# TencentARC/TVTS

Measured on AMD Instinct MI355X. Metric: video-text pairs/sec/node, TVTSv2 pretrain step, higher is better.
Workload: dtype bf16; 1 GPU; TVTSv2 ViT-B/16 8-frame 224^2, mask 0.5, 32-token captions x4, full pretrain step (fwd+losses+bwd+HF-AdamW); pairs_per_gpu=192, global_batch=192, parallelism=dp1, hip_graph=False

## Files before the change

include/tvts_hip.h:

```cpp
#ifndef TVTS_HIP_H
#define TVTS_HIP_H
#include <hip/hip_runtime_api.h>
#ifdef __cplusplus
extern "C" {
#endif

enum { TVTS_ACT_NONE = 0, TVTS_ACT_QUICK_GELU = 1, TVTS_ACT_GELU_ERF = 2,
       TVTS_GATE_ADD_BF16 = 3  };
enum { TVTS_ATTN_FULL = 0, TVTS_ATTN_SPACE = 1, TVTS_ATTN_TIME = 2, TVTS_ATTN_CLS = 3 };
enum {
    TVTS_GEMM_TILE_128 = 1,
    TVTS_GEMM_TILE_256 = 2,
    TVTS_GEMM_FP8_K32 = 4,
    TVTS_TN_NO_EARLY_DMA = 4,
    TVTS_TN_AFAST_0 = 8,
    TVTS_TN_AFAST_1 = 16,
    TVTS_GEMM_STREAMK = 32,
    TVTS_GEMM_NO_STREAMK = 64,
    TVTS_GEMM_RING = 128,
    TVTS_GEMM_NO_RING = 16384,
    TVTS_GEMM_F32_PATCH = 4194304,
    TVTS_GEMM_CLOCK_SAMPLE = 2097152,
    TVTS_GEMM_SIDE_DERIV = 1048576
};
#define TVTS_GEMM_RING_ROWS(r) ((r) == 128 ? (1 << 16) : (r) == 192 ? (2 << 16) : (r) == 256 ? (3 << 16) : 0)
#define TVTS_GEMM_CUS(n) ((((n) / 8) & 63) << 8)
#define TVTS_TN_SPLITS(s) ((s) << 8)
enum {
    TVTS_ATTN_NO_TR = 1,
    TVTS_ATTN_NO_SHARED = 2,
    TVTS_ATTN_NO_FUSED = 4
};

int tvts_gemm_nt_bf16(const void* A, int lda, const void* B, int ldb, int M, int N, int K, const float* bias,
                      const float* residual, int ldr, int act, void* preact, int ldp, const void* gate_h, int ldh,
                      int gate_act, void* out, int ldc, int out_f32, void* workspace, long workspace_bytes, int opts,
                      hipStream_t stream);
long tvts_gemm_nt_workspace_bytes(void);
int tvts_gemm_nt_select(int M, int N, int opts);
int tvts_gemm_tn_bf16(const void* P, int ldp, const void* Q, int ldq, int M, int Na, int Nb, float* out, int ldo,
                      int accumulate, float* colsum, float* workspace, long workspace_elems, int* counters, int n_counters,
                      int opts, hipStream_t stream);
int tvts_gemm_tn_bf16_grouped(const void* problems, int n, void* table_dev, void* table_host, long table_bytes, int upload,
                              float* workspace, long workspace_elems, int opts, hipStream_t stream);
long tvts_gemm_tn_grouped_table_bytes(int n);
int tvts_gemm_tn_select(int M, int Na, int Nb, int opts);
int tvts_gemm_nt_fp8(const void* A, int lda, const void* B, int ldb, int M, int N, int K, const float* scale_a,
                     int scale_a_rows, const float* scale_b, const float* bias, const float* residual, int ldr, int act, void* preact, int ldp,
                     void* out, int ldc, int out_f32, void* q8out, int ldq8, const float* q8_scale, float* q8_amax, int opts,
                     hipStream_t stream);
int tvts_gemm_nt_fp8_gate(const void* A, int lda, const void* B, int ldb, int M, int N, int K, const float* scale_a,
                          int scale_a_rows, const float* scale_b, const float* bias, const void* gate_h, int ldh, int gate_act,
                          void* out, int ldc, void* q8out, int ldq8, const float* q8_scale, float* q8_amax, int opts,
                          hipStream_t stream);
int tvts_gemm_tn_fp8(const void* P8, int ldp, const void* Q8, int ldq, int M, int Na, int Nb, const float* scale_p,
                     const float* scale_q, float* out, int ldo, int accumulate, float* colsum, float* workspace,
                     long workspace_elems, int opts, hipStream_t stream);
int tvts_amax(const void* x, int is_f32, long ld, int rows, int cols, float* amax, hipStream_t stream);
int tvts_quant_fp8(const void* x, int is_f32, long ld, int rows, int cols, const float* amax, void* out, long ldo,
                   float* scale_out, hipStream_t stream);
int tvts_quant_fp8_multi(const void* table, int n, hipStream_t stream);
int tvts_quant_fp8_rows(const void* x, long ld, int rows, int cols, void* out, long ldo, float* row_scale,
                        const float* tscale, float* amax_acc, hipStream_t stream);
int tvts_fp8_update_scales(float* amax, float* scale, int n, hipStream_t stream);
int tvts_gemm_small_f32(const float* A, long sai, long sak, const float* B, long sbk, long sbj, int M, int N, int K,
                        float alpha, const float* bias, float* C, long ldc, int accumulate, hipStream_t stream);
int tvts_rows_linear_bf16(const void* A, long lda, const void* W, int ldw, int R, int N, int K, const float* bias, const float* residual,
                          int ldr, float* out, int ldo, hipStream_t stream);
int tvts_colsum_bf16(const void* X, int ld, int M, int N, float* out, float* workspace, long workspace_elems, hipStream_t stream);

int tvts_layernorm_fwd(const void* x, int ldx, int x_bf16, const int* rows, const float* gamma, const float* beta, float eps, int M,
                       int W, void* y, int ldy, int y_f32, float* mean, float* rstd, hipStream_t stream);
int tvts_layernorm_fwd_fp8(const void* x, int ldx, int x_bf16, const int* rows, const float* gamma, const float* beta, float eps,
                           int M, int W, void* y, int ldy, void* q8, int ldq, float* row_scale, const float* tscale, float* amax_acc,
                           float* mean, float* rstd, hipStream_t stream);
int tvts_layernorm_bwd(const void* dy, int lddy, int dy_f32, const void* x, int ldx, int x_bf16, const int* rows, const float* mean,
                       const float* rstd, const float* gamma, const void* res1, int res1_bf16, int ldr, const void* res2_bf16, int ldr2,
                       int M, int W, float* dx, int lddx, void* dx_bf16, int lddxb, float* dgamma, float* dbeta,
                       float* workspace, long workspace_elems, hipStream_t stream);
int tvts_layernorm_bwd_fp8(const void* dy, int lddy, const void* x, int ldx, int x_bf16, const float* mean, const float* rstd,
                           const float* gamma, const void* res1, int res1_bf16, int ldr, const void* res2_bf16, int ldr2, int M, int W, float* dx,
                           int lddx, void* dx_bf16, int lddxb, void* q8, int ldq, float* row_scale, const float* tscale, float* amax_acc,
                           float* dgamma, float* dbeta, float* workspace, long workspace_elems, hipStream_t stream);
int tvts_layernorm_fwd_cls(const void* x, int ldx, const float* cls_x, int cls_period, void* x_refresh, const float* gamma,
                           const float* beta, float eps, int M, int W, void* y, int ldy, void* q8, int ldq, float* row_scale,
                           const float* tscale, float* amax_acc, float* mean, float* rstd, hipStream_t stream);
int tvts_layernorm_bwd_cls(const void* dy, int lddy, const void* x, int ldx, const float* cls_x, const float* cls_res1, float* cls_dx,
                           int cls_period, const float* mean, const float* rstd, const float* gamma, const void* res1_bf16, int ldr,
                           const void* res2_bf16, int ldr2, int M, int W, void* dx_bf16, int lddxb, void* q8, int ldq, float* row_scale,
                           const float* tscale, float* amax_acc, float* dgamma, float* dbeta, float* workspace, long workspace_elems,
                           hipStream_t stream);

int tvts_attn_fwd(int mode, const void* qkv, int ld, int B, int heads, int S, int T, int n, int causal, void* out, int ldo,
                  float* lse2, int opts, hipStream_t stream);
int tvts_attn_delta(const void* dO, int lddo, const void* O, int ldo, int rows, int heads, float* delta,
                    hipStream_t stream);
int tvts_attn_bwd_dq(int mode, const void* qkv, int ld, int B, int heads, int S, int T, int n, int causal, const void* dO,
                     int lddo, const float* lse2, const float* delta, void* dqkv, int lddq, int opts, hipStream_t stream);
int tvts_attn_bwd_dkv(int mode, const void* qkv, int ld, int B, int heads, int S, int T, int n, int causal, const void* dO,
                      int lddo, const float* lse2, const float* delta, void* dqkv, int lddq, float* cls_acc, int opts,
                      hipStream_t stream);
int tvts_attn_cls_finalize(const float* cls_acc, int B, int heads, int S, void* dqkv, int lddq, hipStream_t stream);
int tvts_attn_bwd(int mode, const void* qkv, int ld, int B, int heads, int S, int T, int n, int causal, const void* dO,
              int lddo, const void* O, int ldo, const float* lse2, float* delta, void* dqkv, int lddq, float* cls_acc,
              long cls_acc_elems, int opts, hipStream_t stream);
int tvts_attn_fwd_divided(int mode, const void* qkv, int ld, int B, int heads, int S, int T, int n, void* out, int ldo,
                      float* lse2, float* cls_ws, long cls_ws_elems, int opts, hipStream_t stream);
int tvts_attn_fwd_divided_q8(int mode, const void* qkv, int ld, int B, int heads, int S, int T, int n, void* out, int ldo,
                      float* lse2, float* cls_ws, long cls_ws_elems, void* q8out, int ldq8, const float* q8_scale, float* q8_amax,
                      int opts, hipStream_t stream);
int tvts_attn_bwd_q8(int mode, const void* qkv, int ld, int B, int heads, int S, int T, int n, int causal, const void* dO,
              int lddo, const void* O, int ldo, const float* lse2, float* delta, void* dqkv, int lddq, float* cls_acc,
              long cls_acc_elems, void* q8out, int ldq8, const float* q8_scale, float* q8_amax, int opts, hipStream_t stream);

// ... 121 lines not shown
```

tvts_amd/csrc/attention.hip:

```cpp
#include "common.h"
#include <stdlib.h>

enum { MODE_FULL = 0, MODE_SPACE = 1, MODE_TIME = 2, MODE_CLS = 3 };
#ifndef TVTS_DH
#define TVTS_DH 64
#endif
#define DH TVTS_DH
#if TVTS_DH == 64
#define NS_DH dh64
#define ABI(name) tvts_attn_##name
#define VSTRIDE 160
#else
#define NS_DH dh80
#define ABI(name) tvts_attn80_##name
#define VSTRIDE 192
#endif
namespace NS_DH {
constexpr int DT = DH / 16;
constexpr int KS = (DH + 31) / 32;
constexpr int NCH = DH / 8;

struct AttnGeom {
    int B, heads, S, T, n;
    int causal;
// ... 1706 lines not shown
                    for (int ks = 0; ks < KS; ++ks) sc = __builtin_amdgcn_mfma_f32_16x16x32_bf16(kc[t][ks], qc[qt][ks], sc, 0, 0, 0);
#pragma unroll
                    for (int e = 0; e < 4; ++e) {
                        const int key = t * 16 + gq * 4 + e;
                        const bool ok = key < m && !(key == 0 && qj == 0 && !first);
                        const float v = ok ? sc[e] * g.scale2 : -INFINITY;
                        st[t][e] = v;
                        mx = fmaxf(mx, v);
                    }
                }
            }
            mx = group_max(mx);
            float rs = 0.f;
#pragma unroll
            for (int t = 0; t < 2 * NU; ++t)
#pragma unroll
                for (int e = 0; e < 4; ++e) {
                    const float pp = __builtin_amdgcn_exp2f(st[t][e] - mx);
                    st[t][e] = pp;
                    rs += pp;
                }
            const float l = group_sum(rs);
            f32x4 o[DT];
#pragma unroll
            for (int dt = 0; dt < DT; ++dt) o[dt] = (f32x4){0, 0, 0, 0};
#pragma unroll
            for (int u = 0; u < NU; ++u) {
                bf16x8 pf;
#pragma unroll
                for (int j = 0; j < 8; ++j) pf[j] = (bf16)st[2 * u + (j >> 2)][j & 3];
#pragma unroll
                for (int dt = 0; dt < DT; ++dt)
                    o[dt] = __builtin_amdgcn_mfma_f32_16x16x32_bf16(frag_T_lim<TR>(Vs, u, dt, lane, RA, RS), pf, o[dt], 0, 0, 0);
            }
            {
                const float inv = 1.0f / l;
                f32x4 on[DT];
#pragma unroll
                for (int dt = 0; dt < DT; ++dt) on[dt] = o[dt] * inv;
                store_tile_rows(opatch, on, lane, [&](int rr) -> bf16* {
                    const int j = qt * 16 + rr;
                    return (j >= 1 && j < m) ? out + (size_t)k_row<MODE_TIME>(g, r, j) * ldo + hcol : nullptr; }, &q8o);
            }
            if (qj >= 1 && qj < m && gq == 0) lse2[(size_t)k_row<MODE_TIME>(g, r, qj) * g.heads + r.h] = mx + log2f(l);
            if (qt == 0) {
                const float Mn = fmaxf(Mr, mx);
                const float a = __builtin_amdgcn_exp2f(Mr - Mn), b = __builtin_amdgcn_exp2f(mx - Mn);
                Lr = Lr * a + l * b;
#pragma unroll
                for (int dt = 0; dt < DT; ++dt) Or[dt] = Or[dt] * a + o[dt] * b;
                Mr = Mn;
            }
        }
    }
    q8o.finish(g, lane);
    float* cst = (float*)(smem + wave * WB + TB);
    if (li == 0) {
        if (gq == 0) { cst[0] = Mr; cst[1] = Lr; }
#pragma unroll
        for (int dt = 0; dt < DT; ++dt)
#pragma unroll
            for (int e = 0; e < 4; ++e) cst[2 + dt * 16 + gq * 4 + e] = Or[dt][e];
    }
    __syncthreads();
    if (threadIdx.x < DH) {
        const int d = threadIdx.x;
        float M = -1e30f;
#pragma unroll
        for (int w = 0; w < 4; ++w) M = fmaxf(M, *(const float*)(smem + w * WB + TB));
        float L = 0.f, O = 0.f;
#pragma unroll
        for (int w = 0; w < 4; ++w) {
            const float* cw = (const float*)(smem + w * WB + TB);
            const float sc = __builtin_amdgcn_exp2f(cw[0] - M);
            L += cw[1] * sc;
            O += cw[2 + d] * sc;
        }
        float* cp = cls_part + ((size_t)(r.b * g.heads + r.h) * chunks + c) * (DH + 2);
        if (d == 0) { cp[0] = M; cp[1] = L; }
        cp[2 + d] = O;
    }
}

template <int MT, bool TR>
__global__ __launch_bounds__(256) void attn_fwd_seq_fused_kernel(AttnGeom g, const bf16* __restrict__ qkv,
                                                                 bf16* __restrict__ out, int ldo, float* __restrict__ lse2) {
    extern __shared__ __attribute__((aligned(16))) char smem[];
    constexpr int RA = MT * 16, TB = RA * VSTRIDE, NU = (MT + 1) / 2;
    constexpr int WB = TB + 1024;
    constexpr int PT = (RA * NCH + 63) / 64;
    const int lane = threadIdx.x & 63, wave = threadIdx.x >> 6;
    char* Vs = smem + wave * WB;
    char* opatch = Vs + TB;
    const int gq = lane >> 4, li = lane & 15;
    const int m = g.S, groups = g.B * g.heads, stride = gridDim.x * 4;
    const bool causal = g.causal != 0;

    bf16x8 qf[MT][KS], kf[MT][KS], vst[PT];
    auto issue = [&](int gid) {
        const bf16* base = qkv + (size_t)(gid / g.heads) * g.S * g.ld + (gid % g.heads) * DH;
#pragma unroll
        for (int t = 0; t < MT; ++t) {
            const int j = t * 16 + li;
            const bf16* rowp = base + (size_t)(j < m ? j : m - 1) * g.ld;
            ld_frags(rowp, gq, qf[t]);
            ld_frags(rowp + g.W, gq, kf[t]);
        }
#pragma unroll
        for (int i = 0; i < PT; ++i) {
            const int cc = lane + 64 * i, row = cc / NCH, ch = cc % NCH;
            vst[i] = row < m ? ldg8(base + (size_t)row * g.ld + 2 * g.W + ch * 8) : zero8();
        }
    };
    int gid = blockIdx.x * 4 + wave;
    if (gid < groups) issue(gid);
    for (; gid < groups; gid += stride) {
#pragma unroll
        for (int i = 0; i < PT; ++i) {
            const int cc = lane + 64 * i, row = cc / NCH, ch = cc % NCH;
            if (row < RA) *(bf16x8*)(Vs + row * VSTRIDE + ch * 16) = vst[i];
        }
        bf16x8 qc[MT][KS], kc[MT][KS];
#pragma unroll
        for (int t = 0; t < MT; ++t)
#pragma unroll
            for (int ks = 0; ks < KS; ++ks) { qc[t][ks] = qf[t][ks]; kc[t][ks] = kf[t][ks]; }
        if (gid + stride < groups) issue(gid + stride);
        const int h = gid % g.heads;
        const size_t row0 = (size_t)(gid / g.heads) * g.S;
        const int hcol = h * DH;
#pragma unroll
        for (int qt = 0; qt < MT; ++qt) {
            const int qj = qt * 16 + li;
            f32x4 st[2 * NU];
            float mx = -INFINITY;
#pragma unroll
            for (int t = 0; t < 2 * NU; ++t) {
                st[t] = (f32x4){-INFINITY, -INFINITY, -INFINITY, -INFINITY};
                if (t < MT) {
                    f32x4 sc = {0, 0, 0, 0};
#pragma unroll
                    for (int ks = 0; ks < KS; ++ks) sc = __builtin_amdgcn_mfma_f32_16x16x32_bf16(kc[t][ks], qc[qt][ks], sc, 0, 0, 0);
#pragma unroll
                    for (int e = 0; e < 4; ++e) {
                        const int key = t * 16 + gq * 4 + e;
                        const bool ok = key < m && !(causal && key > qj);
                        const float v = ok ? sc[e] * g.scale2 : -INFINITY;
                        st[t][e] = v;
                        mx = fmaxf(mx, v);
                    }
                }
            }
            mx = group_max(mx);
            float rs = 0.f;
#pragma unroll
            for (int t = 0; t < 2 * NU; ++t)
#pragma unroll
                for (int e = 0; e < 4; ++e) {
                    const float pp = __builtin_amdgcn_exp2f(st[t][e] - mx);
                    st[t][e] = pp;
                    rs += pp;
                }
            const float l = group_sum(rs);
            f32x4 o[DT];
#pragma unroll
            for (int dt = 0; dt < DT; ++dt) o[dt] = (f32x4){0, 0, 0, 0};
// ... 162 lines not shown
                        }
                    } else {
#pragma unroll
                        for (int e = 0; e < 4; ++e) { pf[t * 4 + e] = (bf16)0.f; dsf[t * 4 + e] = (bf16)0.f; }
                    }
                }
#pragma unroll
                for (int dt = 0; dt < DT; ++dt) {
                    dv[dt] = __builtin_amdgcn_mfma_f32_16x16x32_bf16(frag_T_lim<TR>(Ds, u, dt, lane, RA), pf, dv[dt], 0, 0, 0);
                    dk[dt] = __builtin_amdgcn_mfma_f32_16x16x32_bf16(frag_T_lim<TR>(Qs, u, dt, lane, RA), dsf, dk[dt], 0, 0, 0);
                }
            }
            auto krowp = [&](int third) {
                return [&, third](int rr) -> bf16* {
                    const int j = kt * 16 + rr;
                    return j < m ? dqkv + (row0 + j) * lddq + third * g.W + hcol : nullptr; };
            };
            store_tile_rows(opatch, dk, lane, krowp(1));
            store_tile_rows(opatch, dv, lane, krowp(2));
        }
    }
}

__global__ void attn_cls_merge_kernel(const float* __restrict__ cls_part, int G, int heads, int S, bf16* __restrict__ out,
                                      int ldo, float* __restrict__ lse2, unsigned char* __restrict__ q8 = nullptr,
                                      const float* __restrict__ q8_scale = nullptr, float* __restrict__ q8_amax = nullptr) {
    const int bh = blockIdx.x, d = threadIdx.x;
    const bool live = d < DH;
    float ax = 0.f;
    if (live) {
        const float* cp = cls_part + (size_t)bh * G * (DH + 2);
        float M = -1e30f;
        for (int i = 0; i < G; ++i) M = fmaxf(M, cp[(size_t)i * (DH + 2)]);
        float L = 0.f, O = 0.f;
        for (int i = 0; i < G; ++i) {
            const float sc = __builtin_amdgcn_exp2f(cp[(size_t)i * (DH + 2)] - M);
            L += cp[(size_t)i * (DH + 2) + 1] * sc;
            O += cp[(size_t)i * (DH + 2) + 2 + d] * sc;
        }
        const int b = bh / heads, h = bh % heads;
        const size_t row = (size_t)b * S;
        const bf16 ov = (bf16)(O / L);
        out[row * ldo + h * DH + d] = ov;
        if (q8) {
            const float sc = q8_scale[0], x = (float)ov;
            const int pk = __builtin_amdgcn_cvt_pk_fp8_f32(fminf(fmaxf(x * (sc > 0.f ? 1.0f / sc : 1.0f), -448.0f), 448.0f), 0.f, 0, false);
            q8[row * ldo + h * DH + d] = (unsigned char)(pk & 0xff);
            ax = fabsf(x);
        }
        if (d == 0) lse2[row * heads + h] = M + log2f(L);
    }
    if (q8) amax_publish(q8_amax, wave_max(ax), threadIdx.x & 63);
}

__global__ void attn_cls_finalize_kernel(const float* __restrict__ cls_acc, int B, int heads, int S, int W, int with_q,
                                         bf16* __restrict__ dqkv, int lddq, int parts, unsigned char* __restrict__ q8 = nullptr,
                                         const float* __restrict__ q8_scale = nullptr, float* __restrict__ q8_amax = nullptr) {
    const int idx = blockIdx.x * blockDim.x + threadIdx.x;
    const int d = idx % DH, slot = (idx / DH) % 3, h = (idx / (3 * DH)) % heads, b = idx / (3 * DH * heads);
    const bool live = idx < B * heads * 3 * DH && !(slot == 2 && !with_q);
    float ax = 0.f;
    if (live) {
        const int third = slot == 2 ? 0 : 1 + slot;
        const float* src = cls_acc + ((size_t)(b * heads + h) * parts * 3 + slot) * DH + d;
        float v = 0.f;
        for (int pidx = 0; pidx < parts; ++pidx) v += src[(size_t)pidx * 3 * DH];
        const bf16 ov = (bf16)v;
        dqkv[(size_t)(b * S) * lddq + third * W + h * DH + d] = ov;
        if (q8) {
            const float sc = q8_scale[0], x = (float)ov;
            const int pk = __builtin_amdgcn_cvt_pk_fp8_f32(fminf(fmaxf(x * (sc > 0.f ? 1.0f / sc : 1.0f), -448.0f), 448.0f), 0.f, 0, false);
            q8[(size_t)(b * S) * lddq + third * W + h * DH + d] = (unsigned char)(pk & 0xff);
            ax = fabsf(x);
        }
    }
    if (q8) amax_publish(q8_amax, wave_max(ax), threadIdx.x & 63);
}

}
using namespace NS_DH;

#define ATTN_OPTS(opts)                                                                      \
    const bool use_tr = !((opts) & 1), shared = !((opts) & 2), fused = !((opts) & 4);        \
    (void)use_tr; (void)shared; (void)fused

static int make_geom(AttnGeom& g, int mode, int B, int heads, int S, int T, int n, int causal, int ld) {
    if (B <= 0 || heads <= 0 || S <= 0 || ld % 8) return TVTS_EINVAL;
    if ((mode == MODE_SPACE || mode == MODE_TIME) && (T <= 0 || n <= 0 || S != 1 + T * n)) return TVTS_EINVAL;
    if (mode < MODE_FULL || mode > MODE_CLS) return TVTS_EINVAL;
    g.B = B; g.heads = heads; g.S = S; g.T = T; g.n = n; g.causal = causal; g.ld = ld; g.W = heads * DH; g.kv_len = nullptr;
    g.cls_nq = 1; g.cls_q0 = 0; g.cls_qpos = nullptr; g.cls_parts = 0;
    g.drop_thr = 0; g.drop_inv = 1.f; g.drop_seed = nullptr; g.drop_site = 0;
    g.q8_ref = nullptr; g.q8 = nullptr; g.q8_scale = nullptr; g.q8_amax = nullptr;
    g.scale = 1.0f / sqrtf((float)DH);
    g.scale2 = g.scale * 1.4426950408889634f;
    g.q8_only = 0;
    g.ablate = 0;
    return TVTS_OK;
}
static int items_q(const AttnGeom& g, int mode) {
    const int nq = mode == MODE_SPACE ? g.n : mode == MODE_TIME ? g.T : mode == MODE_CLS ? 1 : g.S;
    const int groups = mode == MODE_SPACE ? g.B * g.heads * g.T : mode == MODE_TIME ? g.B * g.heads * g.n : g.B * g.heads;
    return groups * ceil_div(nq, 16);
}
static int items_k(const AttnGeom& g, int mode) {
    const int nk = mode == MODE_SPACE ? g.n + 1 : mode == MODE_TIME ? g.T + 1 : g.S;
    const int groups = mode == MODE_SPACE ? g.B * g.heads * g.T : mode == MODE_TIME ? g.B * g.heads * g.n : g.B * g.heads;
    return groups * ceil_div(nk, 16);
}

#define DISPATCH_MODE(KERNEL, mode, ...)                                                        \
    do {                                                                                        \
        if (use_tr) {                                                                         \
            switch (mode) {                                                                     \
                case MODE_FULL: hipLaunchKernelGGL((KERNEL<MODE_FULL, true>), __VA_ARGS__); break;   \
                case MODE_SPACE: hipLaunchKernelGGL((KERNEL<MODE_SPACE, true>), __VA_ARGS__); break; \
                case MODE_TIME: hipLaunchKernelGGL((KERNEL<MODE_TIME, true>), __VA_ARGS__); break;   \
                case MODE_CLS: hipLaunchKernelGGL((KERNEL<MODE_CLS, true>), __VA_ARGS__); break;     \
                default: return TVTS_EINVAL;                                                    \
            }                                                                                   \
        } else {                                                                                \
            switch (mode) {                                                                     \
                case MODE_FULL: hipLaunchKernelGGL((KERNEL<MODE_FULL, false>), __VA_ARGS__); break;   \
                case MODE_SPACE: hipLaunchKernelGGL((KERNEL<MODE_SPACE, false>), __VA_ARGS__); break; \
                case MODE_TIME: hipLaunchKernelGGL((KERNEL<MODE_TIME, false>), __VA_ARGS__); break;   \
                case MODE_CLS: hipLaunchKernelGGL((KERNEL<MODE_CLS, false>), __VA_ARGS__); break;     \
                default: return TVTS_EINVAL;                                                    \
            }                                                                                   \
        }                                                                                       \
    } while (0)

struct DropArgs { float p; const unsigned long long* seed; unsigned long long site; };
static int set_drop(AttnGeom& g, const DropArgs* d) {
    if (!d || d->p <= 0.f) return TVTS_OK;
    if (d->p >= 1.f || !d->seed) return TVTS_EINVAL;
    g.drop_thr = (unsigned)((double)d->p * 4294967296.0);
    g.drop_inv = 1.0f / (1.0f - d->p);
    g.drop_seed = d->seed;
    g.drop_site = d->site;
    return TVTS_OK;
}

static int fwd_impl(int mode, const void* qkv, int ld, int B, int heads, int S, int T, int n, int causal, const int* kv_len,
                    void* out, int ldo, float* lse2, int opts, hipStream_t stream, const DropArgs* drop = nullptr) {
    ATTN_OPTS(opts);
    AttnGeom g;
    int rc = make_geom(g, mode, B, heads, S, T, n, causal, ld);
    if (rc) return rc;
    if (ldo % 4 || (kv_len && mode != MODE_FULL)) return TVTS_EINVAL;
    g.kv_len = kv_len;
    if ((rc = set_drop(g, drop))) return rc;
    if (g.drop_thr) {
        if (mode != MODE_FULL) return TVTS_EINVAL;
        const int nb = g.B * g.heads * ceil_div(ceil_div(g.S, 16), 4);
        hipLaunchKernelGGL((attn_fwd_shared_kernel<MODE_FULL, true, true>), dim3(nb), dim3(256), 0, stream, g, (const bf16*)qkv, (bf16*)out, ldo, lse2);
        TVTS_LAUNCH_CHECK();
        return TVTS_OK;
    }
    if (fused && use_tr && mode == MODE_FULL && !kv_len && S <= 32) {
        const int MT = ceil_div(S, 16), groups = B * heads;
        const int lds_bytes = 4 * (MT * 16 * VSTRIDE + 1024);
        const int blocks = ceil_div(groups, 4) < 1536 ? ceil_div(groups, 4) : 1536;
        if (MT == 1) hipLaunchKernelGGL((attn_fwd_seq_fused_kernel<1, true>), dim3(blocks), dim3(256), lds_bytes, stream, g, (const bf16*)qkv, (bf16*)out, ldo, lse2);
        else hipLaunchKernelGGL((attn_fwd_seq_fused_kernel<2, true>), dim3(blocks), dim3(256), lds_bytes, stream, g, (const bf16*)qkv, (bf16*)out, ldo, lse2);
        TVTS_LAUNCH_CHECK();
        return TVTS_OK;
    }
// ... 310 lines not shown
            blocks = B * heads * T; threads = FUSED_THREADS; slot = MT;
        } else {
            const int MT = (T + 1 + 15) / 16, RA = MT * 16;
            const int RS = (MT == 2 && T + 1 <= 20) ? 20 : RA;
            lds_bytes = 4 * (4 * RS * VSTRIDE + 2 * RA * 4 + 3 * DH * 4 + 1024);
            kern = MT == 1 ? attn_bwd_time_fused_kernel<1, true> : RS == 20 ? attn_bwd_time_fused_kernel<2, true, 20> : attn_bwd_time_fused_kernel<2, true>;
            blocks = B * heads * ceil_div(n, TIME_CHUNK); threads = 256; slot = FUSED_MAX_TILES + MT;
        }
        (void)slot;
        if (hipFuncSetAttribute((const void*)kern, hipFuncAttributeMaxDynamicSharedMemorySize, lds_bytes) != hipSuccess)
            return TVTS_EINVAL;
        hipLaunchKernelGGL(kern, dim3(blocks), dim3(threads), lds_bytes, stream, g, (const bf16*)qkv, (const bf16*)dO, lddo,
                           lse2, delta, (bf16*)dqkv, lddq, cls_acc);
        TVTS_LAUNCH_CHECK();
        const int total = B * heads * 3 * DH;
        hipLaunchKernelGGL(attn_cls_finalize_kernel, dim3(ceil_div(total, 256)), dim3(256), 0, stream, cls_acc, B, heads, S,
                           heads * DH, 1, (bf16*)dqkv, lddq, g.cls_parts ? g.cls_parts : 1, g.q8, g.q8_scale, g.q8_amax);
        TVTS_LAUNCH_CHECK();
        return TVTS_OK;
    }
    if (q8out) return TVTS_EINVAL;
    rc = ABI(delta)(dO, lddo, O, ldo, B * S, heads, delta, stream);
    if (rc) return rc;
    rc = ABI(bwd_dq)(mode, qkv, ld, B, heads, S, T, n, causal, dO, lddo, lse2, delta, dqkv, lddq, opts, stream);
    if (rc) return rc;
    rc = ABI(bwd_dkv)(mode, qkv, ld, B, heads, S, T, n, causal, dO, lddo, lse2, delta, dqkv, lddq, cls_acc, opts, stream);
    if (rc) return rc;
    if (divided) {
        rc = ABI(bwd_dq)(MODE_CLS, qkv, ld, B, heads, S, T, n, 0, dO, lddo, lse2, delta, dqkv, lddq, opts, stream);
        if (rc) return rc;
        rc = ABI(cls_finalize)(cls_acc, B, heads, S, dqkv, lddq, stream);
    }
    return rc;
}
extern "C" int ABI(bwd)(int mode, const void* qkv, int ld, int B, int heads, int S, int T, int n, int causal,
                        const void* dO, int lddo, const void* O, int ldo, const float* lse2, float* delta, void* dqkv,
                        int lddq, float* cls_acc, long cls_acc_elems, int opts, hipStream_t stream) {
    return bwd_impl(mode, qkv, ld, B, heads, S, T, n, causal, dO, lddo, O, ldo, lse2, delta, dqkv, lddq, cls_acc, cls_acc_elems,
                    nullptr, 0, nullptr, nullptr, opts, stream);
}
extern "C" int ABI(bwd_q8)(int mode, const void* qkv, int ld, int B, int heads, int S, int T, int n, int causal,
                           const void* dO, int lddo, const void* O, int ldo, const float* lse2, float* delta, void* dqkv,
                           int lddq, float* cls_acc, long cls_acc_elems, void* q8out, int ldq8, const float* q8_scale,
                           float* q8_amax, int opts, hipStream_t stream) {
    if (!q8out) return TVTS_EINVAL;
    return bwd_impl(mode, qkv, ld, B, heads, S, T, n, causal, dO, lddo, O, ldo, lse2, delta, dqkv, lddq, cls_acc, cls_acc_elems,
                    q8out, ldq8, q8_scale, q8_amax, opts, stream);
}

static int fwd_divided_impl(int mode, const void* qkv, int ld, int B, int heads, int S, int T, int n, void* out, int ldo,
                            float* lse2, float* cls_ws, long cls_ws_elems, void* q8out, int ldq8, const float* q8_scale,
                            float* q8_amax, int opts, hipStream_t stream) {
    if (mode != MODE_SPACE && mode != MODE_TIME) return TVTS_EINVAL;
    ATTN_OPTS(opts);
    AttnGeom g;
    int rc = make_geom(g, mode, B, heads, S, T, n, 0, ld);
    if (rc) return rc;
    if (ldo % 4) return TVTS_EINVAL;
    if (q8out) {
        if (ldq8 != ldo || ldo % 8 || !q8_scale) return TVTS_EINVAL;
        g.q8_ref = (const bf16*)out; g.q8 = (unsigned char*)q8out; g.q8_scale = q8_scale; g.q8_amax = q8_amax;
        g.q8_only = (opts & 128) ? 1 : 0;
    }
    const bool fs = fused && use_tr && mode == MODE_SPACE && n + 1 <= FUSED_MAX_TILES * 16;
    const bool ft = fused && use_tr && mode == MODE_TIME && T + 1 <= 32;
    const int G = mode == MODE_SPACE ? T : ceil_div(n, TIME_CHUNK);
    if ((fs || ft) && cls_ws && cls_ws_elems >= (long)B * heads * G * (DH + 2)) {
        typedef void (*Kern)(AttnGeom, const bf16*, bf16*, int, float*, float*);
        Kern kern = nullptr;
        int lds_bytes, blocks;
        if (fs) {
            const int MT = (n + 1 + 15) / 16;
            switch (MT) {
                case 1: kern = attn_fwd_space_fused_kernel<1, true>; break;
                case 2: kern = attn_fwd_space_fused_kernel<2, true>; break;
                case 3: kern = attn_fwd_space_fused_kernel<3, true>; break;
                case 4: kern = attn_fwd_space_fused_kernel<4, true>; break;
                case 5: kern = attn_fwd_space_fused_kernel<5, true>; break;
                case 6: kern = attn_fwd_space_fused_kernel<6, true>; break;
                default: kern = attn_fwd_space_fused_kernel<7, true>; break;
            }
            lds_bytes = 2 * MT * 16 * VSTRIDE + 4 * 1024;
            blocks = B * heads * T;
        } else {
            const int MT = (T + 1 + 15) / 16;
            const int RS = (MT == 2 && T + 1 <= 20) ? 20 : MT * 16;
            kern = MT == 1 ? attn_fwd_time_fused_kernel<1, true> : RS == 20 ? attn_fwd_time_fused_kernel<2, true, 20> : attn_fwd_time_fused_kernel<2, true>;
            lds_bytes = 4 * (RS * VSTRIDE + (DH + 4) * 4 + 1024);
            blocks = B * heads * G;
        }
        hipLaunchKernelGGL(kern, dim3(blocks), dim3(256), lds_bytes, stream, g, (const bf16*)qkv, (bf16*)out, ldo, lse2, cls_ws);
        TVTS_LAUNCH_CHECK();
        hipLaunchKernelGGL(attn_cls_merge_kernel, dim3(B * heads), dim3(DH <= 64 ? 64 : 128), 0, stream, cls_ws, G, heads, S,
                           (bf16*)out, ldo, lse2, g.q8, g.q8_scale, g.q8_amax);
        TVTS_LAUNCH_CHECK();
        return TVTS_OK;
    }
    if (q8out) return TVTS_EINVAL;
    rc = ABI(fwd)(mode, qkv, ld, B, heads, S, T, n, 0, out, ldo, lse2, opts, stream);
    if (rc) return rc;
    return ABI(fwd)(MODE_CLS, qkv, ld, B, heads, S, T, n, 0, out, ldo, lse2, opts, stream);
}
extern "C" int ABI(fwd_divided)(int mode, const void* qkv, int ld, int B, int heads, int S, int T, int n, void* out, int ldo,
                                float* lse2, float* cls_ws, long cls_ws_elems, int opts, hipStream_t stream) {
    return fwd_divided_impl(mode, qkv, ld, B, heads, S, T, n, out, ldo, lse2, cls_ws, cls_ws_elems, nullptr, 0, nullptr, nullptr, opts, stream);
}
extern "C" int ABI(fwd_divided_q8)(int mode, const void* qkv, int ld, int B, int heads, int S, int T, int n, void* out, int ldo,
                                   float* lse2, float* cls_ws, long cls_ws_elems, void* q8out, int ldq8, const float* q8_scale,
                                   float* q8_amax, int opts, hipStream_t stream) {
    if (!q8out) return TVTS_EINVAL;
    return fwd_divided_impl(mode, qkv, ld, B, heads, S, T, n, out, ldo, lse2, cls_ws, cls_ws_elems, q8out, ldq8, q8_scale, q8_amax, opts, stream);
}
```

tvts_amd/hip.py:

```python
from __future__ import annotations

import ctypes
import os
from typing import Optional

import torch

from . import _lib

GEMM_PROFILE = None
HBM_PROFILE = None


class _hbm:

    def __init__(self, family, nbytes):
        self.family, self.nbytes = family, nbytes

    def __enter__(self):
        if HBM_PROFILE is not None:
            self.e0, self.e1 = Event(), Event()
            self.e0.record()

    def __exit__(self, *exc):
        if HBM_PROFILE is not None and exc[0] is None:
            self.e1.record()
            HBM_PROFILE.append((self.family, float(self.nbytes() if callable(self.nbytes) else self.nbytes), self.e0, self.e1))
        return False


def _nb(*tensors_rows):
    return sum(r * t.shape[-1] * t.element_size() for t, r in tensors_rows if t is not None)

ACT = {"none": 0, None: 0, "quick_gelu": 1, "gelu": 2, "add": 3}
MODE = {"full": 0, "space": 1, "time": 2, "cls": 3}


class HipError(RuntimeError):
    pass


def _chk(rc: int, name: str):
    if rc != 0:
        raise HipError(f"{name} failed with code {rc}")


def _p(t: Optional[torch.Tensor]):
    if t is None:
        return None
    if not t.is_cuda:
        raise HipError("tvts_amd kernels need GPU tensors (no CPU path)")
    return ctypes.c_void_p(t.data_ptr())


def _stream():
    return ctypes.c_void_p(torch.cuda.current_stream().cuda_stream)


def _ld(t: torch.Tensor) -> int:
    assert t.dim() == 2 and t.stride(1) == 1, "expected a row-major 2-D tensor"
    return t.stride(0)


_DEFAULTS = dict(nt_tile=0, nt_cus=0, nt_f32_patch=False, nt_streamk=None, tn_streamk=None, fp8_k32=False, tn_tile=0, tn_splits=0, tn_early_dma=None, tn_a_fast=None,
                 attn_tr=True, attn_shared=True, attn_fused=True, attn_ablate=0)
_OPTS = dict(_DEFAULTS)
if os.environ.get("TVTS_NT_F32_PATCH") == "1":
    _OPTS["nt_f32_patch"] = True


class options:

    def __init__(self, **kw):
        bad = set(kw) - set(_DEFAULTS)
        if bad:
            raise KeyError(f"unknown dispatch option(s) {sorted(bad)}")
        self.kw = kw

    def __enter__(self):
        self.saved = dict(_OPTS)
        _OPTS.update(self.kw)
        return self

    def __exit__(self, *exc):
        _OPTS.clear()
        _OPTS.update(self.saved)
        return False


def set_default(**kw):
    bad = set(kw) - set(_DEFAULTS)
    if bad:
        raise KeyError(f"unknown dispatch option(s) {sorted(bad)}")
    _OPTS.update(kw)


def _tile_bits(t):
    return {0: 0, None: 0, 128: 1, 256: 2, "ring": 1 | 128, "ring2": 1 | 128 | (1 << 16), "ring3": 1 | 128 | (2 << 16), "ring4": 1 | 128 | (3 << 16), "noring": 16384,
            "128noring": 1 | 16384}[t]


def _sk_bits(sk):
    return 0 if sk is None else (32 if sk else 64)


def nt_opts(tile=None, cus=None, fp8_k32=None, streamk=None, side_deriv=False):
    tile = _OPTS["nt_tile"] if tile is None else tile
    cus = _OPTS["nt_cus"] if cus is None else cus
    k32 = _OPTS["fp8_k32"] if fp8_k32 is None else fp8_k32
    streamk = _OPTS["nt_streamk"] if streamk is None else streamk
    return (_tile_bits(tile) | (4 if k32 else 0) | (((int(cus) // 8) & 63) << 8) | _sk_bits(streamk) | ((1 << 20) if side_deriv else 0)
            | ((1 << 22) if _OPTS["nt_f32_patch"] else 0))


def tn_opts(tile=None, splits=None, early_dma=None, a_fast=None, streamk=None):
    streamk = _OPTS["tn_streamk"] if streamk is None else streamk
    tile = _OPTS["tn_tile"] if tile is None else tile
    splits = _OPTS["tn_splits"] if splits is None else splits
    early_dma = _OPTS["tn_early_dma"] if early_dma is None else early_dma
    a_fast = _OPTS["tn_a_fast"] if a_fast is None else a_fast
    o = _tile_bits(tile) | (int(splits) << 8) | _sk_bits(streamk)
    if early_dma is not None and not early_dma:
        o |= 4
    if a_fast is not None:
        o |= 16 if a_fast else 8
    return o


def attn_opts(tr=None, shared=None, fused=None, ablate=None, q8_only=False):
    tr = _OPTS["attn_tr"] if tr is None else tr
    shared = _OPTS["attn_shared"] if shared is None else shared
    fused = _OPTS["attn_fused"] if fused is None else fused
    ablate = _OPTS["attn_ablate"] if ablate is None else ablate
    return (0 if tr else 1) | (0 if shared else 2) | (0 if fused else 4) | ((int(ablate) & 7) << 4) | (128 if q8_only else 0)


def gemm_nt_select(M, N, tile=None):
    return _lib.load().tvts_gemm_nt_select(M, N, nt_opts(tile=tile))


def gemm_tn_select(M, Na, Nb, tile=None):
    return _lib.load().tvts_gemm_tn_select(M, Na, Nb, tn_opts(tile=tile))


STREAMK_TAKEN = [0]
NT_WORKSPACE = {}


def _nt_workspace(dev):
    key = (dev, current_lane())
    ws = NT_WORKSPACE.get(key)
    if ws is None:
        ws = NT_WORKSPACE[key] = torch.zeros(_lib.load().tvts_gemm_nt_workspace_bytes(), dtype=torch.uint8, device=dev)
    return ws


def gemm_nt(a, b, out, *, M=None, bias=None, residual=None, act=None, preact=None, gate_h=None, gate_act=None, tile=None, cus=None,
            streamk=None, workspace=True, side_deriv=False):
    lib = _lib.load()
    ws = _nt_workspace(a.device) if workspace else None
    M = a.shape[0] if M is None else M
    N, K = b.shape
    assert a.dtype == torch.bfloat16 and b.dtype == torch.bfloat16 and a.shape[1] == K
    assert out.shape[1] == N and out.dtype in (torch.bfloat16, torch.float32)
    if residual is not None and residual.dtype == torch.bfloat16:
        assert gate_h is None and act is None
        gate_h, gate_act, residual = residual, "add", None
    if GEMM_PROFILE is not None:
        ev0, ev1 = Event(), Event()
        ev0.record()
    cp = CLOCK_PROBE
    sample = (cp is not None and ws is not None and cp["i"] < cp["buf"].shape[0] and out.dtype == torch.bfloat16
              and residual is None and act is None and gate_h is None and M >= 65536)
    if sample:
        zero_(ws[-32:])
    def launch(sk):
        return lib.tvts_gemm_nt_bf16(_p(a), _ld(a), _p(b), _ld(b), M, N, K, _p(bias), _p(residual),
                                     _ld(residual) if residual is not None else 0, ACT[act], _p(preact),
                                     _ld(preact) if preact is not None else 0, _p(gate_h),
                                     _ld(gate_h) if gate_h is not None else 0, ACT[gate_act], _p(out), _ld(out),
                                     1 if out.dtype == torch.float32 else 0, _p(ws), ws.numel() if ws is not None else 0,
                                     nt_opts(tile, cus, streamk=sk, side_deriv=side_deriv) | ((1 << 21) if sample else 0), _stream())
    want_sk = _OPTS["nt_streamk"] if streamk is None else streamk
    rc = launch(streamk)
    if rc == -22 and want_sk and streamk is None:
        rc = launch(False)
    elif rc == 0 and want_sk:
        STREAMK_TAKEN[0] += 1
    _chk(rc, "tvts_gemm_nt_bf16")
    if GEMM_PROFILE is not None:
        ev1.record()
        GEMM_PROFILE.append(("gemm_nt", 2.0 * M * N * K, ev0, ev1, (M, N, K, "f32" if out.dtype == torch.float32 else "bf16", "res" if residual is not None else "", str(act or ""), "gate" if gate_h is not None else "")))
    if sample:
        cp["buf"][cp["i"]].copy_(ws[-32:].view(torch.int64))
        cp["shape"].append((M, N, K))
        cp["i"] += 1


def quantize_fp8(x, q=None, scale=None, amax=None, amax_given=False):
    lib = _lib.load()
    assert x.dim() == 2 and x.stride(1) == 1 and x.dtype in (torch.bfloat16, torch.float32)
    assert not (amax_given and amax is None)
    amax = torch.empty(1, dtype=torch.float32, device=x.device) if amax is None else amax
    scale = torch.empty(1, dtype=torch.float32, device=x.device) if scale is None else scale
    q = torch.empty(x.shape, dtype=torch.uint8, device=x.device) if q is None else q
    f32 = 1 if x.dtype == torch.float32 else 0
    if not amax_given:
        _chk(lib.tvts_amax(_p(x), f32, x.stride(0), x.shape[0], x.shape[1], _p(amax), _stream()), "tvts_amax")
    _chk(lib.tvts_quant_fp8(_p(x), f32, x.stride(0), x.shape[0], x.shape[1], _p(amax), _p(q), q.stride(0), _p(scale), _stream()),
         "tvts_quant_fp8")
    return q, scale


def quantize_fp8_multi_table(entries, device):
    import numpy as np
    rec = np.zeros(len(entries), dtype=[("w", "<u8"), ("q", "<u8"), ("wt", "<u8"), ("qt", "<u8"), ("amax", "<u8"), ("scale", "<u8"),
                                        ("scale_t", "<u8"), ("rows", "<i4"), ("cols", "<i4")])
# ... 726 lines not shown
```

Measured before the change: 1387 pairs/s.

## Pack multiple spatial positions per MFMA tile in fused time-attention forward

Adds a fused time-attention forward kernel that packs 16/T spatial positions' T-frame sequences into a single 16-row MFMA tile with block-diagonal masking. Their CLS-key contribution is handled analytically, and the CLS query's online-softmax partials are accumulated per chunk. With T=8 this fills MFMA tiles that were mostly padding in the per-position kernel (T+1 rows padded to 16 or 32). It is on by default for power-of-two T up to 16, with an env/option to disable it. The cost is extra masking, shuffle reductions and more complex code.

```diff
diff --git a/include/tvts_hip.h b/include/tvts_hip.h
--- a/include/tvts_hip.h
+++ b/include/tvts_hip.h
@@ -29,7 +29,8 @@
 enum {
     TVTS_ATTN_NO_TR = 1,
     TVTS_ATTN_NO_SHARED = 2,
-    TVTS_ATTN_NO_FUSED = 4
+    TVTS_ATTN_NO_FUSED = 4,
+    TVTS_ATTN_UNPACKED = 8
 };
 
 int tvts_gemm_nt_bf16(const void* A, int lda, const void* B, int ldb, int M, int N, int K, const float* bias,
diff --git a/tvts_amd/csrc/attention.hip b/tvts_amd/csrc/attention.hip
--- a/tvts_amd/csrc/attention.hip
+++ b/tvts_amd/csrc/attention.hip
@@ -1812,6 +1812,203 @@
     }
 }
 
+template <bool TR>
+__global__ __launch_bounds__(256, DH == 64 ? 3 : 2) void attn_fwd_time_packed_kernel(AttnGeom g, const bf16* __restrict__ qkv,
+                                                                   bf16* __restrict__ out, int ldo, float* __restrict__ lse2,
+                                                                   float* __restrict__ cls_part) {
+    extern __shared__ __attribute__((aligned(16))) char smem[];
+    constexpr int TB = 16 * VSTRIDE;
+    constexpr int WB = TB + (DH + 2 + 2) * 4 + 1024;
+    constexpr int PT = (16 * NCH + 63) / 64;
+    const int lane = threadIdx.x & 63, wave = threadIdx.x >> 6;
+    char* Vs = smem + wave * WB;
+    char* opatch = Vs + TB + (DH + 4) * 4;
+    const int chunks = (g.n + TIME_CHUNK - 1) / TIME_CHUNK;
+    Grp r;
+    r.h = blockIdx.x % g.heads;
+    const int c = (blockIdx.x / g.heads) % chunks;
+    r.b = blockIdx.x / (g.heads * chunks);
+    const int p_beg = c * TIME_CHUNK;
+    const int p_end = (c + 1) * TIME_CHUNK < g.n ? (c + 1) * TIME_CHUNK : g.n;
+    const int tsh = __builtin_ctz(g.T), tm1 = g.T - 1, GP = 16 >> tsh;
+    const int ntiles = (p_end - p_beg + GP - 1) / GP;
+    const int gq = lane >> 4, li = lane & 15;
+    const int hcol = r.h * DH;
+    const int cls_row = r.b * g.S;
+    const int my_g = li >> tsh, my_f = li & tm1;
+    auto row_of = [&](int p0, int rr) {
+        const int s = p0 + (rr >> tsh);
+        return cls_row + 1 + (rr & tm1) * g.n + (s < p_end ? s : p_end - 1);
+    };
+    bf16x8 qcf[KS], kcf[KS];
+    ld_frags(qkv + (size_t)cls_row * g.ld + hcol, gq, qcf);
+    ld_frags(qkv + (size_t)cls_row * g.ld + g.W + hcol, gq, kcf);
+    f32x4 vc[DT];
+#pragma unroll
+    for (int dt = 0; dt < DT; ++dt) {
+        const bf16x4 t = *(const bf16x4*)(qkv + (size_t)cls_row * g.ld + 2 * g.W + hcol + dt * 16 + gq * 4);
+        vc[dt] = (f32x4){(float)t[0], (float)t[1], (float)t[2], (float)t[3]};
+    }
+    float Mr = -1e30f, Lr = 0.f;
+    float Oc[KS][8];
+#pragma unroll
+    for (int ks = 0; ks < KS; ++ks)
+#pragma unroll
+        for (int j = 0; j < 8; ++j) Oc[ks][j] = 0.f;
+    Q8Out q8o;
+    q8o.init(g);
+
+    bf16x8 qf[KS], kf[KS], vst[PT];
+    auto issue = [&](int p0) {
+        const bf16* rowp = qkv + (size_t)row_of(p0, li) * g.ld + hcol;
+        ld_frags(rowp, gq, qf);
+        ld_frags(rowp + g.W, gq, kf);
+#pragma unroll
+        for (int i = 0; i < PT; ++i) {
+            const int cc = lane + 64 * i, row = cc / NCH, ch = cc % NCH;
+            vst[i] = row < 16 ? ldg8(qkv + (size_t)row_of(p0, row) * g.ld + 2 * g.W + hcol + ch * 8) : zero8();
+        }
+    };
+    int it = wave;
+    if (it < ntiles) issue(p_beg + it * GP);
+    for (; it < ntiles; it += 4) {
+        const int p0 = p_beg + it * GP;
+#pragma unroll
+        for (int i = 0; i < PT; ++i) {
+            const int cc = lane + 64 * i, row = cc / NCH, ch = cc % NCH;
+            if (row < 16) *(bf16x8*)(Vs + row * VSTRIDE + ch * 16) = vst[i];
+        }
+        bf16x8 qc[KS], kc[KS];
+#pragma unroll
+        for (int ks = 0; ks < KS; ++ks) { qc[ks] = qf[ks]; kc[ks] = kf[ks]; }
+        if (it + 4 < ntiles) issue(p_beg + (it + 4) * GP);
+        const bool valid = p0 + my_g < p_end;
+
+        f32x4 sc = {0, 0, 0, 0};
+#pragma unroll
+        for (int ks = 0; ks < KS; ++ks) sc = __builtin_amdgcn_mfma_f32_16x16x32_bf16(kc[ks], qc[ks], sc, 0, 0, 0);
+        float dq = 0.f, dk = 0.f;
+#pragma unroll
+        for (int ks = 0; ks < KS; ++ks)
+#pragma unroll
+            for (int j = 0; j < 8; ++j) {
+                dq += (float)qc[ks][j] * (float)kcf[ks][j];
+                dk += (float)kc[ks][j] * (float)qcf[ks][j];
+            }
+        const float s0 = group_sum(dq) * g.scale2;
+        const float sk = group_sum(dk) * g.scale2;
+
+        float st[4], mx = s0;
+#pragma unroll
+        for (int e = 0; e < 4; ++e) {
+            const bool ok = ((gq * 4 + e) >> tsh) == my_g;
+            st[e] = ok ? sc[e] * g.scale2 : -INFINITY;
+            mx = fmaxf(mx, st[e]);
+        }
+        mx = group_max(mx);
+        const float pc = __builtin_amdgcn_exp2f(s0 - mx);
+        float rs = 0.f;
+        bf16x8 pf;
+#pragma unroll
+        for (int e = 0; e < 4; ++e) {
+            const float pp = __builtin_amdgcn_exp2f(st[e] - mx);
+            rs += pp;
+            pf[e] = (bf16)pp;
+            pf[4 + e] = (bf16)0.f;
+        }
+        const float l = group_sum(rs) + pc;
+        f32x4 o[DT];
+#pragma unroll
+        for (int dt = 0; dt < DT; ++dt) {
+            o[dt] = __builtin_amdgcn_mfma_f32_16x16x32_bf16(frag_T_lim<TR>(Vs, 0, dt, lane, 16), pf, (f32x4){0, 0, 0, 0}, 0, 0, 0);
+            o[dt] += pc * vc[dt];
+        }
+        {
+            const float inv = 1.0f / l;
+            f32x4 on[DT];
+#pragma unroll
+            for (int dt = 0; dt < DT; ++dt) on[dt] = o[dt] * inv;
+            store_tile_rows(opatch, on, lane, [&](int rr) -> bf16* {
+                return p0 + (rr >> tsh) < p_end ? out + (size_t)row_of(p0, rr) * ldo + hcol : nullptr; }, &q8o);
+        }
+        if (valid && gq == 0) lse2[(size_t)(cls_row + 1 + my_f * g.n + p0 + my_g) * g.heads + r.h] = mx + log2f(l);
+
+        const float skm = valid ? sk : -INFINITY;
+        float scc = -INFINITY;
+        if (p0 == 0) {
+            float d = 0.f;
+#pragma unroll
+            for (int ks = 0; ks < KS; ++ks)
+#pragma unroll
+                for (int j = 0; j < 8; ++j) d += (float)qcf[ks][j] * (float)kcf[ks][j];
+            scc = group_sum(d) * g.scale2;
+        }
+        float tmx = fmaxf(skm, scc);
+#pragma unroll
+        for (int s = 1; s < 16; s <<= 1) tmx = fmaxf(tmx, __shfl_xor(tmx, s, 64));
+        const float Mn = fmaxf(Mr, tmx);
+        const float a = __builtin_amdgcn_exp2f(Mr - Mn), pk = __builtin_amdgcn_exp2f(skm - Mn);
+        Lr = Lr * a + pk;
+#pragma unroll
+        for (int ks = 0; ks < KS; ++ks) {
+            const bf16x8 vf = frag_row(Vs, li, ks, gq);
+#pragma unroll
+            for (int j = 0; j < 8; ++j) Oc[ks][j] = Oc[ks][j] * a + pk * (float)vf[j];
+        }
+        if (p0 == 0) {
+            bf16x8 vcf[KS];
+            ld_frags(qkv + (size_t)cls_row * g.ld + 2 * g.W + hcol, gq, vcf);
+            const float pcc = __builtin_amdgcn_exp2f(scc - Mn);
+            if (li == 0) {
+                Lr += pcc;
+#pragma unroll
+                for (int ks = 0; ks < KS; ++ks)
+#pragma unroll
+                    for (int j = 0; j < 8; ++j) Oc[ks][j] += pcc * (float)vcf[ks][j];
+            }
+        }
+        Mr = Mn;
+    }
+    q8o.finish(g, lane);
+#pragma unroll
+    for (int s = 1; s < 16; s <<= 1) {
+        Lr += __shfl_xor(Lr, s, 64);
+#pragma unroll
+        for (int ks = 0; ks < KS; ++ks)
+#pragma unroll
+            for (int j = 0; j < 8; ++j) Oc[ks][j] += __shfl_xor(Oc[ks][j], s, 64);
+    }
+    float* cst = (float*)(smem + wave * WB + TB);
+    if (li == 0) {
+        if (gq == 0) { cst[0] = Mr; cst[1] = Lr; }
+#pragma unroll
+        for (int ks = 0; ks < KS; ++ks)
+#pragma unroll
+            for (int j = 0; j < 8; ++j) {
+                const int d = ks * 32 + gq * 8 + j;
+                if (d < DH) cst[2 + d] = Oc[ks][j];
+            }
+    }
+    __syncthreads();
+    if (threadIdx.x < DH) {
+        const int d = threadIdx.x;
+        float M = -1e30f;
+#pragma unroll
+        for (int w = 0; w < 4; ++w) M = fmaxf(M, *(const float*)(smem + w * WB + TB));
+        float L = 0.f, O = 0.f;
+#pragma unroll
+        for (int w = 0; w < 4; ++w) {
+            const float* cw = (const float*)(smem + w * WB + TB);
+            const float sc = __builtin_amdgcn_exp2f(cw[0] - M);
+            L += cw[1] * sc;
+            O += cw[2 + d] * sc;
+        }
+        float* cp = cls_part + ((size_t)(r.b * g.heads + r.h) * chunks + c) * (DH + 2);
+        if (d == 0) { cp[0] = M; cp[1] = L; }
+        cp[2 + d] = O;
+    }
+}
+
 template <int MT, bool TR>
 __global__ __launch_bounds__(256) void attn_fwd_seq_fused_kernel(AttnGeom g, const bf16* __restrict__ qkv,
                                                                  bf16* __restrict__ out, int ldo, float* __restrict__ lse2) {
@@ -2140,7 +2337,8 @@
 
 #define ATTN_OPTS(opts)                                                                      \
     const bool use_tr = !((opts) & 1), shared = !((opts) & 2), fused = !((opts) & 4);        \
-    (void)use_tr; (void)shared; (void)fused
+    const bool packed = !((opts) & 8);                                                       \
+    (void)use_tr; (void)shared; (void)fused; (void)packed
 
 static int make_geom(AttnGeom& g, int mode, int B, int heads, int S, int T, int n, int causal, int ld) {
     if (B <= 0 || heads <= 0 || S <= 0 || ld % 8) return TVTS_EINVAL;
@@ -2617,6 +2815,10 @@
             }
             lds_bytes = 2 * MT * 16 * VSTRIDE + 4 * 1024;
             blocks = B * heads * T;
+        } else if (packed && T <= 16 && !(T & (T - 1))) {
+            kern = attn_fwd_time_packed_kernel<true>;
+            lds_bytes = 4 * (16 * VSTRIDE + (DH + 4) * 4 + 1024);
+            blocks = B * heads * G;
         } else {
             const int MT = (T + 1 + 15) / 16;
             const int RS = (MT == 2 && T + 1 <= 20) ? 20 : MT * 16;
diff --git a/tvts_amd/hip.py b/tvts_amd/hip.py
--- a/tvts_amd/hip.py
+++ b/tvts_amd/hip.py
@@ -63,10 +63,12 @@
 
 
 _DEFAULTS = dict(nt_tile=0, nt_cus=0, nt_f32_patch=False, nt_streamk=None, tn_streamk=None, fp8_k32=False, tn_tile=0, tn_splits=0, tn_early_dma=None, tn_a_fast=None,
-                 attn_tr=True, attn_shared=True, attn_fused=True, attn_ablate=0)
+                 attn_tr=True, attn_shared=True, attn_fused=True, attn_ablate=0, attn_packed=True)
 _OPTS = dict(_DEFAULTS)
 if os.environ.get("TVTS_NT_F32_PATCH") == "1":
     _OPTS["nt_f32_patch"] = True
+if os.environ.get("TVTS_ATTN_UNPACKED") == "1":
+    _OPTS["attn_packed"] = False
 
 
 class options:
@@ -127,12 +129,14 @@
     return o
 
 
-def attn_opts(tr=None, shared=None, fused=None, ablate=None, q8_only=False):
+def attn_opts(tr=None, shared=None, fused=None, ablate=None, q8_only=False, packed=None):
     tr = _OPTS["attn_tr"] if tr is None else tr
     shared = _OPTS["attn_shared"] if shared is None else shared
     fused = _OPTS["attn_fused"] if fused is None else fused
     ablate = _OPTS["attn_ablate"] if ablate is None else ablate
-    return (0 if tr else 1) | (0 if shared else 2) | (0 if fused else 4) | ((int(ablate) & 7) << 4) | (128 if q8_only else 0)
+    packed = _OPTS["attn_packed"] if packed is None else packed
+    return ((0 if tr else 1) | (0 if shared else 2) | (0 if fused else 4) | (0 if packed else 8) | ((int(ablate) & 7) << 4)
+            | (128 if q8_only else 0))
 
 
 def gemm_nt_select(M, N, tile=None):
```

New measurement: 1389 pairs/s (median of 6 runs). About the same (+0.2%).
